# ShenhanQian/GaussianAvatars

Measured on NVIDIA H100. Metric: rasterizer fwd+bwd frames/sec @100k splats 1080p, higher is better.
Workload: dtype f32

## Files before the change

gaussianavatars_b200/build.py:

```python
from __future__ import annotations

import os
import subprocess
import sys
from concurrent.futures import ThreadPoolExecutor

HERE = os.path.dirname(os.path.abspath(__file__))
CSRC = os.path.join(HERE, "csrc")
LIB = os.path.join(HERE, "libgaussianavatars_b200.so")
OBJ_DIR = os.path.join(HERE, "csrc", "_obj")

ARCH = ["-gencode", "arch=compute_90a,code=sm_90a"]
COMMON = ["-O3", "-std=c++17", "-lineinfo", "-Xcompiler", "-fPIC", "--expt-relaxed-constexpr"]
SOURCES = {
    "api.cu": [],
    "preprocess.cu": ["--fmad=false"],
    "preprocess_bwd.cu": [],
    "binning.cu": [],
    "tile_sort.cu": [],
    "densify.cu": [],
    "regularize.cu": [],
    "nvls.cu": [],
    "blend.cu": [],
    "face_frame.cu": [],
    "flame.cu": [],
    "loss.cu": [],
    "metrics.cu": [],
    "mesh.cu": ["--fmad=false"],
    "optim.cu": [],
}


def _nvcc():
    for cand in (os.environ.get("NVCC"), "/usr/local/cuda/bin/nvcc", "nvcc"):
        if cand and (os.path.isabs(cand) and os.path.exists(cand) or not os.path.isabs(cand)):
            return cand
    return "nvcc"


def _newest_header():
    inc = [os.path.join(CSRC, f) for f in os.listdir(CSRC) if f.endswith((".cuh", ".h", ".inc"))]
    inc.append(os.path.join(HERE, "..", "include", "gab200_rasterizer.h"))
    return max(os.path.getmtime(p) for p in inc)


def build_native(force: bool = False, verbose: bool = False) -> str:
    os.makedirs(OBJ_DIR, exist_ok=True)
    hdr_time = _newest_header()
    jobs = []
    for src, extra in SOURCES.items():
        s = os.path.join(CSRC, src)
        o = os.path.join(OBJ_DIR, src.replace(".cu", ".o"))
        stale = force or not os.path.exists(o) or os.path.getmtime(o) < max(os.path.getmtime(s), hdr_time)
        if stale:
            cmd = [_nvcc(), *ARCH, *COMMON, *extra, "-ccbin", "/usr/bin/g++", "-c", s, "-o", o]
            if verbose:
                cmd.insert(1, "-Xptxas")
                cmd.insert(2, "-v")
            jobs.append(cmd)

    def run(cmd):
        r = subprocess.run(cmd, capture_output=True, text=True)
        if r.returncode != 0:
            raise RuntimeError("nvcc failed: %s\n%s\n%s" % (" ".join(cmd), r.stdout, r.stderr))
        return r.stderr

    if jobs:
        with ThreadPoolExecutor(max_workers=len(jobs)) as ex:
            for out in ex.map(run, jobs):
                if verbose and out:
                    print(out)
    objs = [os.path.join(OBJ_DIR, s.replace(".cu", ".o")) for s in SOURCES]
# ... 10 lines not shown
```

gaussianavatars_b200/csrc/api.cu:

```cuda
#include <atomic>
#include <chrono>
#include <cstdio>
#include <cstdlib>
#include <cstring>
#include <mutex>
#include <vector>

#include "common.cuh"
#include "kernels.cuh"

namespace gab {
static std::atomic<int64_t> g_launches{0};
void count_launch() { g_launches.fetch_add(1, std::memory_order_relaxed); }

struct SortTempCache {
  int64_t n = -1;
  int bits = -1;
  size_t bytes = 0;
};
static thread_local SortTempCache t_sort_cache[2];
static size_t cached_sort_temp_bytes(int64_t N, int bits) {
  SortTempCache& c = t_sort_cache[bits == 32 ? 0 : 1];
  if (c.bits != bits || N > c.n) {
    const int64_t n_up = N + N / 2 + 1024;
    c.bytes = sort_temp_bytes(n_up, bits);
    c.n = n_up;
    c.bits = bits;
  }
  return c.bytes;
}

struct GeomView {
  SplatRec* rec;
  SplatAux* aux;
  uint32_t* tiles_touched;
  uint32_t* offsets;
  uint8_t* clamped;
  uint32_t* depth_keys[2];
  uint32_t* ids[2];
  void* sortA_temp;
  size_t sortA_temp_bytes;
  float* g2d;
  float* face_scratch;
  void* scan_temp;
  size_t scan_temp_bytes;
  DepthBuckets buckets;
  size_t bucket_clear_bytes;
  size_t bytes;
};
static uint32_t depth_bucket_count(int P) {
  uint32_t nb = 256;
  while (nb < 8192 && (int64_t)nb * 64 < P) nb <<= 1;
  return nb;
}
static GeomView carve_geom(void* base, int P, bool need_backward, size_t sort_temp, int face_rows = -1) {
  GeomView g;
  Carver c(base);
  g.rec = c.take<SplatRec>((size_t)P);
  g.aux = c.take<SplatAux>((size_t)P);
  g.tiles_touched = c.take<uint32_t>((size_t)P);
  g.offsets = c.take<uint32_t>((size_t)P);
  g.clamped = c.take<uint8_t>((size_t)P);
  g.depth_keys[0] = c.take<uint32_t>((size_t)P);
  g.depth_keys[1] = c.take<uint32_t>((size_t)P);
  g.ids[0] = c.take<uint32_t>((size_t)P);
  g.ids[1] = c.take<uint32_t>((size_t)P);
  g.g2d = need_backward ? c.take<float>((size_t)P * GAB_G2D_STRIDE) : nullptr;
  g.face_scratch =
      need_backward ? c.take<float>((size_t)(face_rows < 0 ? P : face_rows) * GAB_FACE_GRAD_STRIDE) : nullptr;
  g.scan_temp_bytes = scan_temp_bytes(P);
  g.scan_temp = c.take<char>(g.scan_temp_bytes);
  {
    DepthBuckets& d = g.buckets;
    d.nb = depth_bucket_count(P);
    uint32_t* head = c.take<uint32_t>((size_t)2 * d.nb + GAB_DEPTH_META_WORDS);
    d.counts = head;
    d.tiles = head ? head + d.nb : nullptr;
    d.meta = head ? head + 2 * d.nb : nullptr;
    g.bucket_clear_bytes = sizeof(uint32_t) * ((size_t)2 * d.nb + GAB_DEPTH_META_WORDS);
    d.start = c.take<uint32_t>((size_t)d.nb);
    d.tile_base = c.take<uint32_t>((size_t)d.nb);
    d.rank = c.take<uint32_t>((size_t)P);
    d.lo = d.hi = 0;
    d.scale = 0.f;
    d.enabled = 0;
  }
  g.sortA_temp_bytes = sort_temp;
  g.sortA_temp = c.take<char>(sort_temp);
  g.bytes = c.bytes();
  return g;
}
struct BinView {
  uint32_t* keys[2];
  uint32_t* vals[2];
  uint8_t* strip_mask;
  void* sort_temp;
  size_t sort_temp_bytes;
  size_t bytes;
};
static BinView carve_binning(void* base, int64_t N, bool need_backward, size_t sort_temp) {
  BinView b;
  Carver c(base);
  const size_t n = (size_t)(N > 0 ? N : 1) + 320;
  b.keys[0] = c.take<uint32_t>(n);
  b.keys[1] = c.take<uint32_t>(n);
  b.vals[0] = c.take<uint32_t>(n);
  b.vals[1] = c.take<uint32_t>(n);
  b.strip_mask = need_backward ? c.take<uint8_t>(n) : nullptr;
  b.sort_temp_bytes = sort_temp;
  b.sort_temp = c.take<char>(sort_temp);
  b.bytes = c.bytes();
  return b;
}
struct ImageView {
  uint2* ranges;
  uint32_t* order;
  uint32_t* order_info;
  uint32_t* tile_count;
  uint32_t* tile_cursor;
  float* final_T;
  uint32_t* n_contrib;
  size_t bytes;
};
static ImageView carve_image(void* base, int W, int H, bool need_backward, int views = 1) {
  ImageView v;
  Carver c(base);
  const int gx = (W + GAB_TILE - 1) / GAB_TILE, gy = (H + GAB_TILE - 1) / GAB_TILE;
  const size_t tiles = (size_t)gx * gy * views;
  v.ranges = c.take<uint2>(tiles + 1);
  v.order = c.take<uint32_t>(tiles);
  v.order_info = c.take<uint32_t>(4);
  v.tile_count = c.take<uint32_t>(tiles);
  v.tile_cursor = c.take<uint32_t>(tiles);
  v.final_T = need_backward ? c.take<float>((size_t)W * H * views) : nullptr;
  v.n_contrib = need_backward ? c.take<uint32_t>((size_t)W * H * views) : nullptr;
  v.bytes = c.bytes();
  return v;
}

struct StageTimer {
  std::atomic<int> enabled{0};
  std::mutex mu;
  struct Pending { int stage; cudaEvent_t a, b; };
  std::vector<Pending> pending;
  std::vector<cudaEvent_t> pool;
  double total_ms[GAB200_NUM_STAGES] = {0};
  int64_t launches[GAB200_NUM_STAGES] = {0};
  cudaEvent_t get() {
    if (!pool.empty()) { cudaEvent_t e = pool.back(); pool.pop_back(); return e; }
    cudaEvent_t e; cudaEventCreate(&e); return e;
  }
};
static StageTimer g_timer;
static thread_local bool t_capturing = false;
struct StageScope {
  int stage; cudaStream_t stream; cudaEvent_t a{}, b{}; bool on;
  StageScope(int st, cudaStream_t s) : stage(st), stream(s), on(g_timer.enabled.load() != 0 && !t_capturing) {
    if (on) {
      std::lock_guard<std::mutex> l(g_timer.mu);
      a = g_timer.get(); b = g_timer.get();
      cudaEventRecord(a, stream);
    }
  }
// ... 192 lines not shown
    GAB_CUDA(cudaMemsetAsync(d.counts, 0, g.bucket_clear_bytes, stream));
    if (f.counting) GAB_CUDA(cudaMemsetAsync(f.iv.tile_count, 0, sizeof(uint32_t) * (size_t)tiles, stream));
    StageScope sc(GAB200_STAGE_PREPROCESS, stream);
    if (f.cameras != nullptr)
      launch_preprocess_views(*a, f.views, f.cameras, g.rec, g.aux, g.tiles_touched, g.depth_keys[0], g.ids[0],
                              g.buckets, f.counting ? f.iv.tile_count : nullptr, f.nb ? g.clamped : nullptr, stream);
    else
      launch_preprocess(*a, g.rec, g.aux, g.tiles_touched, f.nb ? g.clamped : nullptr, g.depth_keys[0], g.ids[0],
                        g.buckets, f.counting ? f.iv.tile_count : nullptr, f.tanfov, stream);
  }
  GAB_STAGE_CHECK(f.dbg, stream);
  if (f.counting && run_preprocess) {
    StageScope sc(GAB200_STAGE_TILE_RANGES, stream);
    f.scan_clamp = capacity > 0 ? capacity : 0xffffffffu;
    launch_tile_scan_order(tiles, f.iv.tile_count, f.scan_clamp, f.iv.ranges, f.iv.tile_cursor, f.iv.order,
                           f.iv.order_info, g.buckets.meta, tune_get(GAB200_TUNE_HEAVY_FWD),
                           tune_get(GAB200_TUNE_HEAVY_BWD), stream);
  }
  {
    StageScope sc(GAB200_STAGE_SCAN, stream);
    if (bucket) {
      launch_depth_bucket_sort(f.P, g.buckets, g.depth_keys[0], g.tiles_touched, g.depth_keys[1], g.ids[1], g.offsets,
                               capacity, a->frame_seq, a->sync_mode == GAB200_SYNC_NONE ? a->overflow_flag : nullptr,
                               stream);
      f.selA = 1;
      f.order_count = g.buckets.meta + GAB200_CTR_NUM_LISTED;
    } else {
      GAB_CUDA(run_sort(g.sortA_temp, g.sortA_temp_bytes, g.depth_keys[0], g.depth_keys[1], g.ids[0], g.ids[1], f.P, 32,
                        &f.selA, stream));
      if (!f.counting)
        GAB_CUDA(run_scan(g.scan_temp, g.scan_temp_bytes, g.ids[f.selA], g.tiles_touched, g.offsets, f.P, stream));
      f.order_count = nullptr;
    }
    if (!bucket)
      launch_publish_counters(g.buckets.meta, f.counting ? nullptr : g.offsets, f.P, capacity, a->frame_seq,
                              a->sync_mode == GAB200_SYNC_NONE ? a->overflow_flag : nullptr, stream);
  }
  GAB_STAGE_CHECK(f.dbg, stream);
  GAB_CUDA(cudaMemcpyAsync(f.ctr_host, g.buckets.meta, sizeof(uint32_t) * GAB200_NUM_COUNTERS, cudaMemcpyDeviceToHost,
                           stream));
  if (f.ctr_event) GAB_CUDA(cudaEventRecord(f.ctr_event, stream));
  return GAB200_OK;
}

void emit(const Frame& f, const uint32_t* offsets, uint32_t cap, uint32_t* cursor, const BinView& bv) {
  if (f.cameras != nullptr)
    launch_emit_keys_views(f.P, f.gx, f.gy, f.g.rec, f.g.aux, f.g.ids[f.selA], offsets, f.order_count, f.g.buckets.meta,
                           cap, cursor, bv.keys[0], bv.vals[0], f.a->exact_binning, f.a->P, f.stream);
  else
    launch_emit_keys(f.P, f.gx, f.gy, f.g.rec, f.g.aux, f.g.ids[f.selA], offsets, f.order_count, f.g.buckets.meta, cap,
                     cursor, bv.keys[0], bv.vals[0], f.a->exact_binning, f.stream);
}

int enqueue_binning_blend(Frame& f, void* bin, int64_t cap, int64_t n_known, size_t sort_temp, bool redo) {
  const gab200_forward_args* a = f.a;
  gab200_frame_state* st = f.st;
  cudaStream_t stream = f.stream;
  const int tiles = f.tiles;
  BinView bv = carve_binning(bin, cap, f.nb, sort_temp);
  st->binning_capacity = cap;
  st->binning_buffer = bin;
  st->binning_bytes = bv.bytes;
  const int64_t n_sort = n_known >= 0 ? n_known : cap;
  const bool counting = f.counting && f.P > 0;
  st->tile_sort_path = counting ? 1 : 0;
  if (bv.strip_mask != nullptr && n_sort > 0) GAB_CUDA(cudaMemsetAsync(bv.strip_mask, 0, (size_t)n_sort, stream));
  int selector = 0;
  if (counting) {
    if (redo) {
      StageScope sc(GAB200_STAGE_TILE_RANGES, stream);
      f.scan_clamp = (uint32_t)(cap < 0xffffffffll ? cap : 0xffffffffll);
      launch_tile_scan_order(tiles, f.iv.tile_count, f.scan_clamp, f.iv.ranges, f.iv.tile_cursor, f.iv.order,
                             f.iv.order_info, f.g.buckets.meta, tune_get(GAB200_TUNE_HEAVY_FWD),
                             tune_get(GAB200_TUNE_HEAVY_BWD), stream);
    }
    if (n_sort > 0) {
      {
        StageScope sc(GAB200_STAGE_EMIT_KEYS, stream);
        emit(f, nullptr, (uint32_t)cap, f.iv.tile_cursor, bv);
      }
      GAB_STAGE_CHECK(f.dbg, stream);
      {
        StageScope sc(GAB200_STAGE_SORT, stream);
        launch_tile_sort(tiles, f.iv.ranges, f.iv.order, f.iv.order_info, bv.keys[0], bv.vals[0], f.g.ids[f.selA],
                         f.order_count, f.P, stream);
      }
      GAB_STAGE_CHECK(f.dbg, stream);
    }
  } else {
    GAB_CUDA(cudaMemsetAsync(f.iv.ranges, 0, sizeof(uint2) * ((size_t)tiles + 1), stream));
    if (n_sort > 0) {
      if (n_known < 0) GAB_CUDA(cudaMemsetAsync(bv.keys[0], 0xff, sizeof(uint32_t) * (size_t)cap, stream));
      {
        StageScope sc(GAB200_STAGE_EMIT_KEYS, stream);
        emit(f, f.g.offsets, (uint32_t)cap, nullptr, bv);
      }
      GAB_STAGE_CHECK(f.dbg, stream);
      {
        StageScope sc(GAB200_STAGE_SORT, stream);
        GAB_CUDA(run_sort(bv.sort_temp, bv.sort_temp_bytes, bv.keys[0], bv.keys[1], bv.vals[0], bv.vals[1], n_sort,
                          st->sort_bits, &selector, stream));
      }
      GAB_STAGE_CHECK(f.dbg, stream);
      {
        StageScope sc(GAB200_STAGE_TILE_RANGES, stream);
        launch_tile_ranges(n_sort, (uint32_t)tiles, bv.keys[selector], f.iv.ranges, stream);
      }
      GAB_STAGE_CHECK(f.dbg, stream);
    }
    StageScope sc(GAB200_STAGE_TILE_RANGES, stream);
    launch_tile_scan_order(tiles, nullptr, 0xffffffffu, f.iv.ranges, nullptr, f.iv.order, f.iv.order_info, nullptr,
                           tune_get(GAB200_TUNE_HEAVY_FWD), tune_get(GAB200_TUNE_HEAVY_BWD), stream);
  }
  st->sorted_selector = selector;
  {
    StageScope sc(GAB200_STAGE_BLEND_FWD, stream);
    if (f.cameras != nullptr && f.nb)
      launch_blend_forward_views_train(f.views, f.W, f.H, f.iv.ranges, f.iv.order, f.iv.order_info, bv.vals[selector],
                                       f.g.rec, a->bg, a->out_color, f.iv.final_T, f.iv.n_contrib, bv.strip_mask,
                                       stream);
    else if (f.cameras != nullptr)
      launch_blend_forward_views(f.views, f.W, f.H, f.iv.ranges, f.iv.order, f.iv.order_info, bv.vals[selector], f.g.rec,
                                 a->bg, a->out_color, f.out_rgb8, stream);
    else
      launch_blend_forward(f.W, f.H, f.iv.ranges, f.iv.order, f.iv.order_info, bv.vals[selector], f.g.rec, a->bg,
                           a->out_color, f.iv.final_T, f.iv.n_contrib, bv.strip_mask, f.out_rgb8, stream);
  }
  GAB_STAGE_CHECK(f.dbg, stream);
  return GAB200_OK;
}

int wait_counters(Frame& f) {
  for (;;) {
    const cudaError_t q = cudaEventQuery(f.ctr_event);
    if (q == cudaSuccess) return GAB200_OK;
    if (q != cudaErrorNotReady) return GAB200_ERR_CUDA;
  }
}
}

static int64_t run_forward(const gab200_forward_args* a, const float* tanfov, uint8_t* out_rgb8,
                           gab200_frame_state* st, void* stream_, int views = 1, const float* cameras = nullptr) {
  cudaStream_t stream = (cudaStream_t)stream_;
  if (!validate(a, out_rgb8 != nullptr && a != nullptr && a->need_backward == 0) || st == nullptr)
    return GAB200_ERR_INVALID_ARGUMENT;
  if (check_arch() < 0) return GAB200_ERR_ARCH;
  memset(st, 0, sizeof(*st));
  Frame f;
  f.a = a; f.tanfov = tanfov; f.out_rgb8 = out_rgb8; f.st = st; f.stream = stream;
  f.P = a->P * views; f.W = a->image_width; f.H = a->image_height;
  f.gx = (f.W + GAB_TILE - 1) / GAB_TILE; f.gy = (f.H + GAB_TILE - 1) / GAB_TILE;
  f.tiles = f.gx * f.gy * views;
  f.views = views; f.cameras = cameras;
  f.nb = a->need_backward != 0;
  f.dbg = a->debug != 0;
  f.counting = tune_get(GAB200_TUNE_TILE_SORT) == 1;
  const int P = f.P;
  const int mode = a->sync_mode;
  const bool speculative = mode != GAB200_SYNC_EXACT;
  if (speculative && P > 0 && a->binning_hint <= 0) return GAB200_ERR_INVALID_ARGUMENT;
  if (mode == GAB200_SYNC_NONE && a->counters_host == nullptr) return GAB200_ERR_INVALID_ARGUMENT;
  cudaStreamCaptureStatus cap_status = cudaStreamCaptureStatusNone;
  GAB_CUDA(cudaStreamIsCapturing(stream, &cap_status));
  if (cap_status != cudaStreamCaptureStatusNone && mode != GAB200_SYNC_NONE) return GAB200_ERR_INVALID_ARGUMENT;
  struct CaptureGuard {
    bool prev;
    explicit CaptureGuard(bool c) : prev(t_capturing) { t_capturing = c; }
    ~CaptureGuard() { t_capturing = prev; }
  } capture_guard(cap_status != cudaStreamCaptureStatusNone);

  const size_t tempA = cached_sort_temp_bytes(P > 0 ? P : 1, 32);
  GeomView gsz = carve_geom(nullptr, P, f.nb, tempA, a->P);
  void* geom = a->alloc_geom(a->alloc_user, gsz.bytes);
  if (geom == nullptr) return GAB200_ERR_ALLOC;
  f.g = carve_geom(geom, P, f.nb, tempA, a->P);
  ImageView isz = carve_image(nullptr, f.W, f.H, f.nb, views);
  void* img = a->alloc_image(a->alloc_user, isz.bytes);
  if (img == nullptr) return GAB200_ERR_ALLOC;
  f.iv = carve_image(img, f.W, f.H, f.nb, views);
  st->geom_buffer = geom; st->geom_bytes = f.g.bytes;
  st->image_buffer = img; st->image_bytes = f.iv.bytes;
  st->sort_bits = (int)tile_bits((uint32_t)f.tiles);
  st->depth_bits = 32;
  st->device_counters = f.g.buckets.meta;
  st->attempts = 1;
  st->depth_key_min = 1; st->depth_key_max = 0;
  st->reserved0 = (cameras != nullptr && f.nb) ? views : 0;

  const double t0 = now_us();
  if (P == 0) {
    BinView bsz = carve_binning(nullptr, 0, f.nb, 0);
    void* bin = a->alloc_binning(a->alloc_user, bsz.bytes);
    if (bin == nullptr) return GAB200_ERR_ALLOC;
    GAB_CUDA(cudaMemsetAsync(f.g.buckets.counts, 0, f.g.bucket_clear_bytes, stream));
    const int rc = enqueue_binning_blend(f, bin, 0, 0, 0, false);
    if (rc < 0) return rc;
    st->num_rendered = st->num_candidates = 0;
    return 0;
  }

  f.ctr_host = a->counters_host;
  f.ctr_event = nullptr;
  if (mode != GAB200_SYNC_NONE) {
    if (!t_slot.ok()) return GAB200_ERR_CUDA;
    f.ctr_event = t_slot.ev;
    if (f.ctr_host == nullptr) f.ctr_host = t_slot.host;
  }
  bool bucket = a->depth_hint_hi > a->depth_hint_lo && tune_get(GAB200_TUNE_DEPTH_SORT) == 0;
  int64_t cap = speculative ? (int64_t)a->binning_hint : 0;
  int rc = enqueue_geometry(f, bucket, true, (uint32_t)cap);
  if (rc < 0) return rc;

  void* bin = nullptr;
  int64_t bin_cap = 0;
  size_t tempB = 0;
  double t_alloc = now_us();
  host_add(0, t_alloc - t0);
  if (a->binning_hint > 0) {
    bin_cap = a->binning_hint;
    tempB = f.counting ? 0 : cached_sort_temp_bytes(bin_cap, st->sort_bits);
    const BinView hv = carve_binning(nullptr, bin_cap, f.nb, tempB);
    bin = a->alloc_binning(a->alloc_user, hv.bytes);
    if (bin == nullptr) return GAB200_ERR_ALLOC;
  }
  double t1 = now_us();
  host_add(2, t1 - t_alloc);
  if (speculative) {
    rc = enqueue_binning_blend(f, bin, cap, -1, tempB, false);
    if (rc < 0) return rc;
    const double t2 = now_us();
    host_add(3, t2 - t1);
    t1 = t2;
  }
  st->depth_sort_path = bucket ? 1 : 0;
  if (mode == GAB200_SYNC_NONE) {
    st->num_rendered = st->num_candidates = -1;
    g_host_ns[5].fetch_add(1, std::memory_order_relaxed);
    return 0;
  }

  rc = wait_counters(f);
  if (rc < 0) return rc;
  bool redo = !speculative;
  if (bucket && f.ctr_host[GAB200_CTR_BUCKET_OVERFLOW] != 0) {
    bucket = false;
    st->depth_sort_path = 2;
    st->attempts++;
    rc = enqueue_geometry(f, false, false, (uint32_t)cap);
    if (rc < 0) return rc;
    rc = wait_counters(f);
    if (rc < 0) return rc;
    redo = true;
  }
  if (f.ctr_host[GAB200_CTR_NUM_RENDERED_HI] != 0) return GAB200_ERR_OVERFLOW;
  const int64_t N = (int64_t)f.ctr_host[GAB200_CTR_NUM_RENDERED];
  st->depth_key_min = ~f.ctr_host[GAB200_CTR_NOT_MIN_DEPTH_KEY];
  st->depth_key_max = f.ctr_host[GAB200_CTR_MAX_DEPTH_KEY];
  st->num_rendered = st->num_candidates = N;
  double t2 = now_us();
  host_add(1, t2 - t1);
  if (speculative && N > cap) {
    redo = true;
    st->attempts++;
  }
  if (redo) {
    if (bin == nullptr || N > bin_cap) {
      bin_cap = N;
      tempB = f.counting ? 0 : cached_sort_temp_bytes(bin_cap > 0 ? bin_cap : 1, st->sort_bits);
      const BinView bsz = carve_binning(nullptr, bin_cap, f.nb, tempB);
      bin = a->alloc_binning(a->alloc_user, bsz.bytes);
      if (bin == nullptr) return GAB200_ERR_ALLOC;
    }
    const double t3 = now_us();
    host_add(2, t3 - t2);
    rc = enqueue_binning_blend(f, bin, bin_cap, N, tempB, speculative);
    if (rc < 0) return rc;
    host_add(3, now_us() - t3);
  }
  g_host_ns[5].fetch_add(1, std::memory_order_relaxed);
  return N;
}

int64_t gab200_forward(const gab200_forward_args* a, gab200_frame_state* st, void* stream) {
  return run_forward(a, nullptr, nullptr, st, stream);
}

int64_t gab200_forward_device_fov(const gab200_forward_args* a, const float* tanfov, gab200_frame_state* st,
                                  void* stream) {
  return run_forward(a, tanfov, nullptr, st, stream);
}

int64_t gab200_forward_display(const gab200_forward_args* a, const float* tanfov, uint8_t* out_rgb8,
                               gab200_frame_state* st, void* stream) {
  return run_forward(a, tanfov, out_rgb8, st, stream);
}

int64_t gab200_forward_views(const gab200_forward_args* a, int32_t views, const float* cameras, uint8_t* out_rgb8,
                             gab200_frame_state* st, void* stream) {
  if (a == nullptr || a->need_backward != 0 || views < 1 || views > 65535 || cameras == nullptr || st == nullptr)
    return GAB200_ERR_INVALID_ARGUMENT;
  gab200_forward_args v = *a;
  v.viewmatrix = v.projmatrix = v.campos = cameras;
  if (!validate(&v, out_rgb8 != nullptr)) return GAB200_ERR_INVALID_ARGUMENT;
  const int64_t view_tiles = (((int64_t)v.image_width + GAB_TILE - 1) / GAB_TILE) *
                             (((int64_t)v.image_height + GAB_TILE - 1) / GAB_TILE);
  if ((int64_t)views * v.P > INT32_MAX || (int64_t)views * view_tiles > INT32_MAX) return GAB200_ERR_INVALID_ARGUMENT;
  return run_forward(&v, nullptr, out_rgb8, st, stream, views, cameras);
}

static bool validate_views_train(const gab200_forward_args* a, int32_t views, const float* cameras,
                                 gab200_forward_args& v) {
  if (a == nullptr || views < 1 || views > 65535 || cameras == nullptr) return false;
  v = *a;
  v.viewmatrix = v.projmatrix = v.campos = cameras;
  v.need_backward = 1;
  if (!validate(&v)) return false;
  if (v.input_mode != GAB200_INPUT_BOUND_RAW || v.colors_precomp != nullptr) return false;
  const int64_t view_tiles = (((int64_t)v.image_width + GAB_TILE - 1) / GAB_TILE) *
                             (((int64_t)v.image_height + GAB_TILE - 1) / GAB_TILE);
  return (int64_t)views * v.P <= INT32_MAX && (int64_t)views * view_tiles <= INT32_MAX;
}
// ... 429 lines not shown
```

gaussianavatars_b200/csrc/kernels.cuh:

```cuda
#pragma once
#include "common.cuh"

namespace gab {

#define SH_C0 0.28209479177387814f
#define SH_C1 0.4886025119029199f
#define SH_C2_0 1.0925484305920792f
#define SH_C2_1 -1.0925484305920792f
#define SH_C2_2 0.31539156525252005f
#define SH_C2_3 -1.0925484305920792f
#define SH_C2_4 0.5462742152960396f
#define SH_C3_0 -0.5900435899266435f
#define SH_C3_1 2.890611442640554f
#define SH_C3_2 -0.4570457994644658f
#define SH_C3_3 0.3731763325901154f
#define SH_C3_4 -0.4570457994644658f
#define SH_C3_5 1.445305721320277f
#define SH_C3_6 -0.5900435899266435f

void count_launch();
int tune_get(int knob);

struct TileSpan {
  bool any, full;
// ... 27 lines not shown
    if (ystar >= lo && ystar <= hi) xl = -dxmax;
    else xl = fminf((-B * lo - hl) / A, (-B * hi - hh) / A);
    const float X0 = px + xl - 0.02f, X1 = px + xr + 0.02f;
    int t0 = (int)ceilf((X0 - (float)(GAB_TILE - 1)) * (1.0f / GAB_TILE));
    int t1 = (int)floorf(X1 * (1.0f / GAB_TILE)) + 1;
    cx0 = min(max(t0, rx0), rx1);
    cx1 = max(min(t1, rx1), cx0);
  }
};

#define GAB_DEPTH_BUCKET_CAP 2048
#define GAB_DEPTH_META_WORDS (GAB200_NUM_COUNTERS + 2)
#define GAB_META_TOTAL64 GAB200_NUM_COUNTERS
struct DepthBuckets {
  uint32_t* counts;
  uint32_t* tiles;
  uint32_t* meta;
  uint32_t* start;
  uint32_t* tile_base;
  uint32_t* rank;
  uint32_t nb;
  uint32_t lo, hi;
  float scale;
  int enabled;
};
__device__ __forceinline__ uint32_t depth_bucket(uint32_t key, const DepthBuckets& d) {
  if (key <= d.lo) return 0u;
  if (key >= d.hi) return d.nb - 1u;
  const uint32_t b = (uint32_t)(__uint2float_rz(key - d.lo) * d.scale);
  return b < d.nb ? b : d.nb - 1u;
}
void launch_preprocess(const gab200_forward_args& a, SplatRec* rec, SplatAux* aux, uint32_t* tiles_touched,
                       uint8_t* clamped, uint32_t* depth_keys, uint32_t* ids, const DepthBuckets& buckets,
                       uint32_t* tile_count, const float* tanfov, cudaStream_t stream);
void launch_preprocess_views(const gab200_forward_args& a, int views, const float* cameras, SplatRec* rec, SplatAux* aux,
                             uint32_t* tiles_touched, uint32_t* depth_keys, uint32_t* ids, const DepthBuckets& buckets,
                             uint32_t* tile_count, uint8_t* clamped, cudaStream_t stream);
void launch_depth_bucket_sort(int P, const DepthBuckets& buckets, const uint32_t* depth_keys,
                              const uint32_t* tiles_touched, uint32_t* scratch_keys, uint32_t* sorted_ids,
                              uint32_t* offsets, uint32_t capacity, uint32_t seq, uint32_t* sticky_overflow,
                              cudaStream_t stream);
void launch_bind_activate(const gab200_forward_args& a, float* means3D, float* opacities, float* scales, float* cov3D,
                          cudaStream_t stream);
void launch_mark_visible(int P, const float* means3D, const float* V, uint8_t* present, cudaStream_t stream);
void launch_publish_counters(uint32_t* counters, const uint32_t* offsets, int P, uint32_t capacity, uint32_t seq,
                             uint32_t* sticky_overflow, cudaStream_t stream);
void launch_emit_keys(int P, int gx, int gy, const SplatRec* rec, const SplatAux* aux, const uint32_t* order,
                      const uint32_t* offsets, const uint32_t* order_count, const uint32_t* counters, uint32_t capacity,
                      uint32_t* cursor, uint32_t* keys, uint32_t* vals, int exact_binning, cudaStream_t stream);
void launch_emit_keys_views(int P, int gx, int gy, const SplatRec* rec, const SplatAux* aux, const uint32_t* order,
                            const uint32_t* offsets, const uint32_t* order_count, const uint32_t* counters, uint32_t cap,
                            uint32_t* cursor, uint32_t* keys, uint32_t* vals, int exact_binning, int view_splats,
                            cudaStream_t stream);
void launch_tile_ranges(int64_t N, uint32_t tiles, const uint32_t* keys, uint2* ranges, cudaStream_t stream);
void launch_expand_keys(int64_t N, const uint32_t* tile_keys, const uint32_t* ids, const SplatAux* aux, uint64_t* out,
                        cudaStream_t stream);
#define GAB_TILE_SORT_SMEM 2048
void launch_tile_scan_order(int tiles, const uint32_t* tile_count, uint32_t clamp, uint2* ranges, uint32_t* cursor,
                            uint32_t* order, uint32_t* order_info, uint32_t* counters, int heavy_fwd, int heavy_bwd,
                            cudaStream_t stream);
void launch_tile_sort(int tiles, const uint2* ranges, const uint32_t* order, const uint32_t* order_info, uint32_t* keys,
                      uint32_t* vals, const uint32_t* rank_to_id, const uint32_t* listed, int P, cudaStream_t stream);
void launch_expand_keys_by_range(int tiles, const uint2* ranges, const uint32_t* ids, const SplatAux* aux, uint64_t* out,
                                 cudaStream_t stream);

size_t scan_temp_bytes(int P);
cudaError_t run_scan(void* temp, size_t temp_bytes, const uint32_t* order, const uint32_t* tiles_touched, uint32_t* out,
                     int P, cudaStream_t stream);
size_t sort_temp_bytes(int64_t N, int end_bit);
cudaError_t run_sort(void* temp, size_t temp_bytes, uint32_t* keys_a, uint32_t* keys_b, uint32_t* vals_a,
                     uint32_t* vals_b, int64_t N, int end_bit, int* selector_out, cudaStream_t stream);

void launch_blend_forward(int W, int H, const uint2* ranges, const uint32_t* order, const uint32_t* order_info,
                          const uint32_t* point_list, const SplatRec* rec,
                          const float* bg, float* out_color, float* final_T, uint32_t* n_contrib, uint8_t* strip_mask,
                          uint8_t* out_rgb8, cudaStream_t stream);
void launch_blend_forward_views(int views, int W, int H, const uint2* ranges, const uint32_t* order,
                                const uint32_t* order_info, const uint32_t* point_list, const SplatRec* rec,
                                const float* bg, float* out_color, uint8_t* out_rgb8, cudaStream_t stream);
void launch_blend_forward_views_train(int views, int W, int H, const uint2* ranges, const uint32_t* order,
                                      const uint32_t* order_info, const uint32_t* point_list, const SplatRec* rec,
                                      const float* bg, float* out_color, float* final_T, uint32_t* n_contrib,
                                      uint8_t* strip_mask, cudaStream_t stream);
void launch_blend_backward(int W, int H, const uint2* ranges, const uint32_t* order, const uint32_t* order_info,
                           const uint32_t* point_list, const SplatRec* rec,
                           const float* bg, const float* final_T, const uint32_t* n_contrib, const float* dL_dpix,
                           const uint8_t* strip_mask, float* g2d, cudaStream_t stream);
void launch_blend_backward_views(int views, int W, int H, const uint2* ranges, const uint32_t* order,
                                 const uint32_t* order_info, const uint32_t* point_list, const SplatRec* rec,
                                 const float* bg, const float* final_T, const uint32_t* n_contrib, const float* dL_dpix,
                                 const uint8_t* strip_mask, float* g2d, cudaStream_t stream);

void launch_preprocess_backward(const gab200_backward_args& b, const SplatRec* rec, const SplatAux* aux,
                                const uint8_t* clamped, const float* g2d, float* face_scratch, const float* tanfov,
                                cudaStream_t stream);
void launch_preprocess_backward_views(const gab200_backward_args& b, int views, const float* cameras,
                                      const SplatAux* aux, const uint8_t* clamped, const float* g2d,
                                      float* face_scratch, cudaStream_t stream);
#define GAB_FACE_GRAD_STRIDE 13

void launch_face_frame_forward(int F, const float* verts, const int32_t* faces, float* fc, float* fR, float* fs,
                               cudaStream_t stream);
void launch_face_frame_backward(int F, const float* verts, const int32_t* faces, const float* g_fc, const float* g_fR,
                                const float* g_fs, float* g_verts, cudaStream_t stream);

void launch_l1_loss_u8(int64_t n, const float* img, const uint8_t* gt, const float* upstream, float* grad, float* loss,
                       cudaStream_t stream);

void launch_photometric_loss(int C, int H, int W, const float* img, const void* gt, int gt_is_u8, float lambda,
                             float* grad, float* loss, float* scratch, cudaStream_t stream);

size_t metrics_scratch_bytes(int H, int W);
void launch_image_metrics(int H, int W, int kind, const void* render, const uint8_t* gt, const int32_t* row, int rows,
                          const int32_t* skip, float* table, void* scratch, cudaStream_t stream);

size_t mesh_scratch_bytes(int F, int W, int H);
cudaError_t launch_mesh_render(const gab200_mesh_args& a, cudaStream_t stream);
// ... 26 lines not shown
```

gaussianavatars_b200/csrc/preprocess.cu:

```cuda
#include "common.cuh"
#include "kernels.cuh"
#include "splat_math.cuh"

namespace gab {

#define REC_SCALE_AC (-0.5f * 1.4426950408889634f)
#define REC_SCALE_B (-1.4426950408889634f)

__device__ __forceinline__ void stage_camera(const gab200_forward_args& a, Camera& cam) {
  int t = threadIdx.x;
  if (t < 16) cam.V[t] = a.viewmatrix[t];
  else if (t < 32) cam.Pm[t - 16] = a.projmatrix[t - 16];
  else if (t < 35) cam.campos[t - 32] = a.campos[t - 32];
  __syncthreads();
}
__device__ __forceinline__ void stage_camera_row(const float* __restrict__ row, Camera& cam) {
  int t = threadIdx.x;
  if (t < 16) cam.V[t] = row[t];
  else if (t < 32) cam.Pm[t - 16] = row[t];
  else if (t < 35) cam.campos[t - 32] = row[t];
  __syncthreads();
}

template <bool BOUND, bool DEVFOV>
// ... 410 lines not shown
                                                              uint32_t* __restrict__ cursor,
                                                              uint32_t* __restrict__ keys, uint32_t* __restrict__ vals,
                                                              int exact_binning, uint32_t view_splats,
                                                              uint32_t view_tiles) {
  emit_keys<true>(P, gx, gy, rec, aux, order, offsets, order_count, counters, cap, cursor, keys, vals, exact_binning,
                  view_splats, view_tiles);
}

__global__ void publish_counters_kernel(uint32_t* __restrict__ counters, const uint32_t* __restrict__ offsets, int P,
                                        uint32_t capacity, uint32_t seq, uint32_t* __restrict__ sticky_overflow) {
  if (P > 0) {
    if (offsets != nullptr) counters[GAB200_CTR_NUM_RENDERED] = offsets[P - 1];
    counters[GAB200_CTR_NUM_LISTED] = (uint32_t)P;
    counters[GAB200_CTR_BUCKET_OVERFLOW] = 0;
  }
  counters[GAB200_CTR_CAPACITY] = capacity;
  counters[GAB200_CTR_SEQ] = seq;
  const uint32_t hi = counters[GAB_META_TOTAL64 + 1];
  counters[GAB200_CTR_NUM_RENDERED_HI] = hi;
  if (sticky_overflow != nullptr &&
      (hi != 0 || counters[GAB200_CTR_BUCKET_OVERFLOW] != 0 || counters[GAB200_CTR_NUM_RENDERED] > capacity))
    *sticky_overflow = 1u;
}
void launch_publish_counters(uint32_t* counters, const uint32_t* offsets, int P, uint32_t capacity, uint32_t seq,
                             uint32_t* sticky_overflow, cudaStream_t stream) {
  publish_counters_kernel<<<1, 1, 0, stream>>>(counters, offsets, P, capacity, seq, sticky_overflow);
  count_launch();
}

void launch_emit_keys(int P, int gx, int gy, const SplatRec* rec, const SplatAux* aux, const uint32_t* order,
                      const uint32_t* offsets, const uint32_t* order_count, const uint32_t* counters, uint32_t cap,
                      uint32_t* cursor, uint32_t* keys, uint32_t* vals, int exact_binning, cudaStream_t stream) {
  const int warps = (P + 31) / 32;
  const int threads = 256, blocks = (warps * 32 + threads - 1) / threads;
  if (blocks == 0) return;
  emit_keys_kernel<<<blocks, threads, 0, stream>>>(P, gx, gy, rec, aux, order, offsets, order_count, counters, cap, cursor,
                                                   keys, vals, exact_binning);
  count_launch();
}

void launch_emit_keys_views(int P, int gx, int gy, const SplatRec* rec, const SplatAux* aux, const uint32_t* order,
                            const uint32_t* offsets, const uint32_t* order_count, const uint32_t* counters, uint32_t cap,
                            uint32_t* cursor, uint32_t* keys, uint32_t* vals, int exact_binning, int view_splats,
                            cudaStream_t stream) {
  const int warps = (P + 31) / 32;
  const int threads = 256, blocks = (warps * 32 + threads - 1) / threads;
  if (blocks == 0) return;
  emit_keys_views_kernel<<<blocks, threads, 0, stream>>>(P, gx, gy, rec, aux, order, offsets, order_count, counters, cap,
                                                         cursor, keys, vals, exact_binning, (uint32_t)view_splats,
                                                         (uint32_t)(gx * gy));
  count_launch();
}

__global__ void __launch_bounds__(256) tile_ranges_kernel(int64_t N, uint32_t tiles, const uint32_t* __restrict__ keys,
                                                          uint2* __restrict__ ranges) {
  const int64_t idx = (int64_t)blockIdx.x * blockDim.x + threadIdx.x;
  if (idx >= N) return;
  const uint32_t cur = min(keys[idx], tiles);
  if (idx == 0)
    ranges[cur].x = 0;
  else {
    const uint32_t prev = min(keys[idx - 1], tiles);
    if (cur != prev) {
      ranges[prev].y = (uint32_t)idx;
      ranges[cur].x = (uint32_t)idx;
    }
  }
  if (idx == N - 1) ranges[cur].y = (uint32_t)N;
}

__global__ void expand_keys_kernel(int64_t N, const uint32_t* __restrict__ tile_keys, const uint32_t* __restrict__ ids,
                                   const SplatAux* __restrict__ aux, uint64_t* __restrict__ out) {
  const int64_t i = (int64_t)blockIdx.x * blockDim.x + threadIdx.x;
  if (i >= N) return;
  out[i] = ((uint64_t)tile_keys[i] << 32) | (uint64_t)__float_as_uint(aux[ids[i]].depth);
}
void launch_expand_keys(int64_t N, const uint32_t* tile_keys, const uint32_t* ids, const SplatAux* aux, uint64_t* out,
                        cudaStream_t stream) {
  if (N == 0) return;
  expand_keys_kernel<<<(unsigned)((N + 255) / 256), 256, 0, stream>>>(N, tile_keys, ids, aux, out);
  count_launch();
}

void launch_tile_ranges(int64_t N, uint32_t tiles, const uint32_t* keys, uint2* ranges, cudaStream_t stream) {
  if (N == 0) return;
  const int threads = 256;
  const int64_t blocks = (N + threads - 1) / threads;
  tile_ranges_kernel<<<(unsigned)blocks, threads, 0, stream>>>(N, tiles, keys, ranges);
  count_launch();
}

}
```

include/gab200_rasterizer.h:

```cpp
#ifndef GAB200_RASTERIZER_H
#define GAB200_RASTERIZER_H

#include <stddef.h>
#include <stdint.h>

#ifdef __cplusplus
extern "C" {
#endif

#define GAB200_ABI_VERSION 3

typedef enum gab200_status {
  GAB200_OK = 0,
  GAB200_ERR_INVALID_ARGUMENT = -1,
  GAB200_ERR_CUDA = -2,
  GAB200_ERR_ALLOC = -3,
  GAB200_ERR_ARCH = -4,
  GAB200_ERR_OVERFLOW = -5
} gab200_status;

typedef enum gab200_input_mode {
  GAB200_INPUT_ACTIVATED = 0,
  GAB200_INPUT_BOUND_RAW = 1
} gab200_input_mode;
// ... 305 lines not shown
int32_t gab200_densify_apply(const gab200_densify_args* args, const gab200_densify_out* out, void* stream);

#define GAB200_FLAME_J 5
#define GAB200_FLAME_POSE_BASIS 36
#define GAB200_FLAME_MAX_EXPR 100
#define GAB200_FLAME_FRAME_FLOATS 128
typedef struct gab200_flame_assets {
  uint32_t abi_version;
  int32_t V, n_shape, n_expr, J;
  int32_t parents[GAB200_FLAME_J];
  const float* v_template;
  const float* shapedirs;
  const float* posedirs;
  const float* J_regressor;
  const float* lbs_weights;
} gab200_flame_assets;

size_t gab200_flame_scratch_bytes(int32_t V, int32_t n_expr);

int32_t gab200_flame_prepare(const gab200_flame_assets* assets, const float* shape, const float* static_offset,
                             void* scratch, void* stream);

typedef struct gab200_flame_frame_args {
  uint32_t abi_version;
  int32_t T;
  const gab200_flame_assets* assets;
  const void* scratch;
  const int32_t* timestep;
  const float* expr;
  const float* rotation;
  const float* neck_pose;
  const float* jaw_pose;
  const float* eyes_pose;
  const float* translation;
  float* frame;
} gab200_flame_frame_args;

int32_t gab200_flame_forward(const gab200_flame_frame_args* args, float* verts, float* verts_cano, void* stream);

typedef struct gab200_flame_grads {
  float* expr;
  float* rotation;
  float* neck_pose;
  float* jaw_pose;
  float* eyes_pose;
  float* translation;
} gab200_flame_grads;
int32_t gab200_flame_backward(const gab200_flame_frame_args* args, const float* dL_dverts, const float* dL_dverts_cano,
                              const gab200_flame_grads* grads, void* stream);

int32_t gab200_export_binning(const gab200_forward_args* args, const gab200_frame_state* state, uint64_t* keys,
                              uint32_t* values, uint32_t* ranges, void* stream);

enum {
  GAB200_STAGE_PREPROCESS = 0,
  GAB200_STAGE_SCAN = 1,
  GAB200_STAGE_EMIT_KEYS = 2,
  GAB200_STAGE_SORT = 3,
  GAB200_STAGE_TILE_RANGES = 4,
  GAB200_STAGE_BLEND_FWD = 5,
  GAB200_STAGE_BLEND_BWD = 6,
  GAB200_STAGE_PREPROCESS_BWD = 7,
  GAB200_NUM_STAGES = 8
};
void gab200_stage_timing_enable(int32_t enable);
void gab200_host_times(double out[6], int32_t reset);
int32_t gab200_stage_times(double total_ms[GAB200_NUM_STAGES], int64_t launches[GAB200_NUM_STAGES], int32_t reset);

enum {
  GAB200_TUNE_HEAVY_FWD = 0,
  GAB200_TUNE_HEAVY_BWD = 1,
  GAB200_TUNE_DEPTH_SORT = 2,
  GAB200_TUNE_TILE_SORT = 4,
  GAB200_TUNE_NVLS_CTAS = 5,
  GAB200_NUM_TUNABLES = 8
};
int32_t gab200_tune(int32_t knob, int32_t value);

int64_t gab200_launch_count(void);

const char* gab200_status_string(int32_t status);
uint32_t gab200_abi_version(void);

#ifdef __cplusplus
}
#endif
#endif
```

Before: 1720.

## Replace CUB tile-key sort with device-count-driven onesweep radix sort

Adds a custom onesweep-style LSD radix sort: one histogram kernel counts all digits, then each pass ranks keys with warp match-any, scatters them locally in shared memory and uses decoupled look-back for global offsets. Every kernel reads the true rendered count from the device counters, so work scales with the actual key count instead of the allocated capacity. This removes the 0xff memset of the key buffer, and the strip-mask clear is folded into the tile-ranges kernel. In exchange, the look-back spin-waits on chunks taken through an atomic counter, and the status scratch grows with capacity.

```diff
diff --git a/gaussianavatars_b200/build.py b/gaussianavatars_b200/build.py
--- a/gaussianavatars_b200/build.py
+++ b/gaussianavatars_b200/build.py
@@ -18,6 +18,7 @@
     "preprocess_bwd.cu": [],
     "binning.cu": [],
     "tile_sort.cu": [],
+    "tile_bin.cu": [],
     "densify.cu": [],
     "regularize.cu": [],
     "nvls.cu": [],
diff --git a/gaussianavatars_b200/csrc/api.cu b/gaussianavatars_b200/csrc/api.cu
--- a/gaussianavatars_b200/csrc/api.cu
+++ b/gaussianavatars_b200/csrc/api.cu
@@ -15,17 +15,15 @@
 
 struct SortTempCache {
   int64_t n = -1;
-  int bits = -1;
   size_t bytes = 0;
 };
-static thread_local SortTempCache t_sort_cache[2];
-static size_t cached_sort_temp_bytes(int64_t N, int bits) {
-  SortTempCache& c = t_sort_cache[bits == 32 ? 0 : 1];
-  if (c.bits != bits || N > c.n) {
+static thread_local SortTempCache t_sort_cache;
+static size_t cached_sort_temp_bytes(int64_t N) {
+  SortTempCache& c = t_sort_cache;
+  if (N > c.n) {
     const int64_t n_up = N + N / 2 + 1024;
-    c.bytes = sort_temp_bytes(n_up, bits);
+    c.bytes = sort_temp_bytes(n_up, 32);
     c.n = n_up;
-    c.bits = bits;
   }
   return c.bytes;
 }
@@ -94,11 +92,10 @@
   uint32_t* keys[2];
   uint32_t* vals[2];
   uint8_t* strip_mask;
-  void* sort_temp;
-  size_t sort_temp_bytes;
+  void* sort_scratch;
   size_t bytes;
 };
-static BinView carve_binning(void* base, int64_t N, bool need_backward, size_t sort_temp) {
+static BinView carve_binning(void* base, int64_t N, bool need_backward, size_t sort_scratch) {
   BinView b;
   Carver c(base);
   const size_t n = (size_t)(N > 0 ? N : 1) + 320;
@@ -107,8 +104,7 @@
   b.vals[0] = c.take<uint32_t>(n);
   b.vals[1] = c.take<uint32_t>(n);
   b.strip_mask = need_backward ? c.take<uint8_t>(n) : nullptr;
-  b.sort_temp_bytes = sort_temp;
-  b.sort_temp = c.take<char>(sort_temp);
+  b.sort_scratch = c.take<char>(sort_scratch);
   b.bytes = c.bytes();
   return b;
 }
@@ -407,21 +403,21 @@
                      cursor, bv.keys[0], bv.vals[0], f.a->exact_binning, f.stream);
 }
 
-int enqueue_binning_blend(Frame& f, void* bin, int64_t cap, int64_t n_known, size_t sort_temp, bool redo) {
+int enqueue_binning_blend(Frame& f, void* bin, int64_t cap, int64_t n_known, size_t sort_scratch, bool redo) {
   const gab200_forward_args* a = f.a;
   gab200_frame_state* st = f.st;
   cudaStream_t stream = f.stream;
   const int tiles = f.tiles;
-  BinView bv = carve_binning(bin, cap, f.nb, sort_temp);
+  BinView bv = carve_binning(bin, cap, f.nb, sort_scratch);
   st->binning_capacity = cap;
   st->binning_buffer = bin;
   st->binning_bytes = bv.bytes;
   const int64_t n_sort = n_known >= 0 ? n_known : cap;
   const bool counting = f.counting && f.P > 0;
   st->tile_sort_path = counting ? 1 : 0;
-  if (bv.strip_mask != nullptr && n_sort > 0) GAB_CUDA(cudaMemsetAsync(bv.strip_mask, 0, (size_t)n_sort, stream));
   int selector = 0;
   if (counting) {
+    if (bv.strip_mask != nullptr && n_sort > 0) GAB_CUDA(cudaMemsetAsync(bv.strip_mask, 0, (size_t)n_sort, stream));
     if (redo) {
       StageScope sc(GAB200_STAGE_TILE_RANGES, stream);
       f.scan_clamp = (uint32_t)(cap < 0xffffffffll ? cap : 0xffffffffll);
@@ -445,7 +441,6 @@
   } else {
     GAB_CUDA(cudaMemsetAsync(f.iv.ranges, 0, sizeof(uint2) * ((size_t)tiles + 1), stream));
     if (n_sort > 0) {
-      if (n_known < 0) GAB_CUDA(cudaMemsetAsync(bv.keys[0], 0xff, sizeof(uint32_t) * (size_t)cap, stream));
       {
         StageScope sc(GAB200_STAGE_EMIT_KEYS, stream);
         emit(f, f.g.offsets, (uint32_t)cap, nullptr, bv);
@@ -453,13 +448,13 @@
       GAB_STAGE_CHECK(f.dbg, stream);
       {
         StageScope sc(GAB200_STAGE_SORT, stream);
-        GAB_CUDA(run_sort(bv.sort_temp, bv.sort_temp_bytes, bv.keys[0], bv.keys[1], bv.vals[0], bv.vals[1], n_sort,
-                          st->sort_bits, &selector, stream));
+        GAB_CUDA(launch_tile_bin_sort(bv.keys, bv.vals, f.g.buckets.meta, n_sort, st->sort_bits, bv.sort_scratch,
+                                      &selector, stream));
       }
       GAB_STAGE_CHECK(f.dbg, stream);
       {
         StageScope sc(GAB200_STAGE_TILE_RANGES, stream);
-        launch_tile_ranges(n_sort, (uint32_t)tiles, bv.keys[selector], f.iv.ranges, stream);
+        launch_tile_bin_ranges(bv.keys[selector], f.g.buckets.meta, n_sort, f.iv.ranges, bv.strip_mask, stream);
       }
       GAB_STAGE_CHECK(f.dbg, stream);
     }
@@ -524,7 +519,7 @@
     ~CaptureGuard() { t_capturing = prev; }
   } capture_guard(cap_status != cudaStreamCaptureStatusNone);
 
-  const size_t tempA = cached_sort_temp_bytes(P > 0 ? P : 1, 32);
+  const size_t tempA = cached_sort_temp_bytes(P > 0 ? P : 1);
   GeomView gsz = carve_geom(nullptr, P, f.nb, tempA, a->P);
   void* geom = a->alloc_geom(a->alloc_user, gsz.bytes);
   if (geom == nullptr) return GAB200_ERR_ALLOC;
@@ -573,7 +568,7 @@
   host_add(0, t_alloc - t0);
   if (a->binning_hint > 0) {
     bin_cap = a->binning_hint;
-    tempB = f.counting ? 0 : cached_sort_temp_bytes(bin_cap, st->sort_bits);
+    tempB = f.counting ? 0 : tile_bin_scratch_bytes(bin_cap, st->sort_bits);
     const BinView hv = carve_binning(nullptr, bin_cap, f.nb, tempB);
     bin = a->alloc_binning(a->alloc_user, hv.bytes);
     if (bin == nullptr) return GAB200_ERR_ALLOC;
@@ -621,7 +616,7 @@
   if (redo) {
     if (bin == nullptr || N > bin_cap) {
       bin_cap = N;
-      tempB = f.counting ? 0 : cached_sort_temp_bytes(bin_cap > 0 ? bin_cap : 1, st->sort_bits);
+      tempB = f.counting ? 0 : tile_bin_scratch_bytes(bin_cap, st->sort_bits);
       const BinView bsz = carve_binning(nullptr, bin_cap, f.nb, tempB);
       bin = a->alloc_binning(a->alloc_user, bsz.bytes);
       if (bin == nullptr) return GAB200_ERR_ALLOC;
diff --git a/gaussianavatars_b200/csrc/kernels.cuh b/gaussianavatars_b200/csrc/kernels.cuh
--- a/gaussianavatars_b200/csrc/kernels.cuh
+++ b/gaussianavatars_b200/csrc/kernels.cuh
@@ -103,7 +103,6 @@
                             const uint32_t* offsets, const uint32_t* order_count, const uint32_t* counters, uint32_t cap,
                             uint32_t* cursor, uint32_t* keys, uint32_t* vals, int exact_binning, int view_splats,
                             cudaStream_t stream);
-void launch_tile_ranges(int64_t N, uint32_t tiles, const uint32_t* keys, uint2* ranges, cudaStream_t stream);
 void launch_expand_keys(int64_t N, const uint32_t* tile_keys, const uint32_t* ids, const SplatAux* aux, uint64_t* out,
                         cudaStream_t stream);
 #define GAB_TILE_SORT_SMEM 2048
@@ -114,6 +113,12 @@
                       uint32_t* vals, const uint32_t* rank_to_id, const uint32_t* listed, int P, cudaStream_t stream);
 void launch_expand_keys_by_range(int tiles, const uint2* ranges, const uint32_t* ids, const SplatAux* aux, uint64_t* out,
                                  cudaStream_t stream);
+
+size_t tile_bin_scratch_bytes(int64_t cap, int bits);
+cudaError_t launch_tile_bin_sort(uint32_t* keys[2], uint32_t* vals[2], const uint32_t* counters, int64_t cap, int bits,
+                                 void* scratch, int* selector_out, cudaStream_t stream);
+void launch_tile_bin_ranges(const uint32_t* keys, const uint32_t* counters, int64_t cap, uint2* ranges,
+                            uint8_t* strip_mask, cudaStream_t stream);
 
 size_t scan_temp_bytes(int P);
 cudaError_t run_scan(void* temp, size_t temp_bytes, const uint32_t* order, const uint32_t* tiles_touched, uint32_t* out,
diff --git a/gaussianavatars_b200/csrc/preprocess.cu b/gaussianavatars_b200/csrc/preprocess.cu
--- a/gaussianavatars_b200/csrc/preprocess.cu
+++ b/gaussianavatars_b200/csrc/preprocess.cu
@@ -486,23 +486,6 @@
   count_launch();
 }
 
-__global__ void __launch_bounds__(256) tile_ranges_kernel(int64_t N, uint32_t tiles, const uint32_t* __restrict__ keys,
-                                                          uint2* __restrict__ ranges) {
-  const int64_t idx = (int64_t)blockIdx.x * blockDim.x + threadIdx.x;
-  if (idx >= N) return;
-  const uint32_t cur = min(keys[idx], tiles);
-  if (idx == 0)
-    ranges[cur].x = 0;
-  else {
-    const uint32_t prev = min(keys[idx - 1], tiles);
-    if (cur != prev) {
-      ranges[prev].y = (uint32_t)idx;
-      ranges[cur].x = (uint32_t)idx;
-    }
-  }
-  if (idx == N - 1) ranges[cur].y = (uint32_t)N;
-}
-
 __global__ void expand_keys_kernel(int64_t N, const uint32_t* __restrict__ tile_keys, const uint32_t* __restrict__ ids,
                                    const SplatAux* __restrict__ aux, uint64_t* __restrict__ out) {
   const int64_t i = (int64_t)blockIdx.x * blockDim.x + threadIdx.x;
@@ -516,12 +499,4 @@
   count_launch();
 }
 
-void launch_tile_ranges(int64_t N, uint32_t tiles, const uint32_t* keys, uint2* ranges, cudaStream_t stream) {
-  if (N == 0) return;
-  const int threads = 256;
-  const int64_t blocks = (N + threads - 1) / threads;
-  tile_ranges_kernel<<<(unsigned)blocks, threads, 0, stream>>>(N, tiles, keys, ranges);
-  count_launch();
-}
-
-}
+}
diff --git a/gaussianavatars_b200/csrc/tile_bin.cu b/gaussianavatars_b200/csrc/tile_bin.cu
--- /dev/null
+++ b/gaussianavatars_b200/csrc/tile_bin.cu
@@ -0,0 +1,255 @@
+#include <algorithm>
+
+#include <cuda/atomic>
+
+#include "common.cuh"
+#include "kernels.cuh"
+
+namespace gab {
+
+#define TB_THREADS 256
+#define TB_WARPS (TB_THREADS / 32)
+#define TB_ITEMS 15
+#define TB_TILE (TB_THREADS * TB_ITEMS)
+#define TB_DIGIT_BITS 8
+#define TB_RADIX (1 << TB_DIGIT_BITS)
+#define TB_MAX_PASSES 4
+#define TB_HEAD_WORDS (TB_MAX_PASSES * TB_RADIX + TB_MAX_PASSES)
+
+static_assert(TB_RADIX == TB_THREADS, "one thread per digit");
+
+#define TB_AGGREGATE (1ull << 32)
+#define TB_INCLUSIVE (2ull << 32)
+
+__device__ __forceinline__ uint32_t tb_count(const uint32_t* counters, uint32_t cap) {
+  if (counters[GAB200_CTR_BUCKET_OVERFLOW] != 0 || counters[GAB200_CTR_NUM_RENDERED_HI] != 0) return 0;
+  return min(counters[GAB200_CTR_NUM_RENDERED], cap);
+}
+
+int tile_bin_passes(int bits) { return (bits + TB_DIGIT_BITS - 1) / TB_DIGIT_BITS; }
+
+int64_t tile_bin_chunks(int64_t cap) { return (cap + TB_TILE - 1) / TB_TILE; }
+
+size_t tile_bin_scratch_bytes(int64_t cap, int bits) {
+  Carver c(nullptr);
+  c.take<uint32_t>(TB_HEAD_WORDS);
+  c.take<unsigned long long>((size_t)tile_bin_passes(bits) * (size_t)tile_bin_chunks(cap) * TB_RADIX);
+  return c.bytes();
+}
+
+__global__ void __launch_bounds__(TB_THREADS) tile_bin_hist_kernel(const uint32_t* __restrict__ keys,
+                                                                   const uint32_t* __restrict__ counters, uint32_t cap,
+                                                                   int passes, uint32_t* __restrict__ hist,
+                                                                   unsigned long long* __restrict__ status,
+                                                                   uint32_t chunks) {
+  __shared__ uint32_t s_hist[TB_MAX_PASSES][TB_RADIX];
+  const uint32_t n = tb_count(counters, cap);
+  const size_t base = (size_t)blockIdx.x * TB_TILE;
+  if (base >= n) return;
+  const int t = threadIdx.x;
+  for (int p = 0; p < passes; p++) {
+    s_hist[p][t] = 0;
+    status[((size_t)p * chunks + blockIdx.x) * TB_RADIX + t] = 0ull;
+  }
+  __syncthreads();
+  const uint32_t valid = (uint32_t)min((size_t)TB_TILE, (size_t)n - base);
+  for (uint32_t j = t; j < valid; j += TB_THREADS) {
+    const uint32_t k = keys[base + j];
+    for (int p = 0; p < passes; p++) atomicAdd(&s_hist[p][(k >> (p * TB_DIGIT_BITS)) & (TB_RADIX - 1)], 1u);
+  }
+  __syncthreads();
+  for (int p = 0; p < passes; p++)
+    if (s_hist[p][t] != 0) atomicAdd(&hist[p * TB_RADIX + t], s_hist[p][t]);
+}
+
+__device__ __forceinline__ void tb_block_scan2(uint32_t& a, uint32_t& b, uint32_t (*s)[TB_WARPS]) {
+  const int lane = threadIdx.x & 31, w = threadIdx.x >> 5;
+  uint32_t ia = a, ib = b;
+#pragma unroll
+  for (int d = 1; d < 32; d <<= 1) {
+    const uint32_t na = __shfl_up_sync(0xffffffffu, ia, d), nb = __shfl_up_sync(0xffffffffu, ib, d);
+    if (lane >= d) { ia += na; ib += nb; }
+  }
+  if (lane == 31) { s[0][w] = ia; s[1][w] = ib; }
+  __syncthreads();
+  uint32_t oa = 0, ob = 0;
+  for (int k = 0; k < w; k++) { oa += s[0][k]; ob += s[1][k]; }
+  a = oa + ia - a;
+  b = ob + ib - b;
+}
+
+__global__ void __launch_bounds__(TB_THREADS) tile_bin_pass_kernel(
+    const uint32_t* __restrict__ keys_in, const uint32_t* __restrict__ vals_in, uint32_t* __restrict__ keys_out,
+    uint32_t* __restrict__ vals_out, const uint32_t* __restrict__ counters, uint32_t cap, int pass,
+    const uint32_t* __restrict__ hist, uint32_t* __restrict__ next_chunk, unsigned long long* __restrict__ status,
+    uint32_t chunks) {
+  __shared__ uint32_t s_warp[TB_WARPS][TB_RADIX];
+  __shared__ uint32_t s_keys[TB_TILE];
+  __shared__ uint32_t s_vals[TB_TILE];
+  __shared__ uint32_t s_local[TB_RADIX];
+  __shared__ uint32_t s_global[TB_RADIX];
+  __shared__ uint32_t s_scan[2][TB_WARPS];
+  __shared__ uint32_t s_chunk;
+  constexpr unsigned FULL = 0xffffffffu;
+  const int t = threadIdx.x, lane = t & 31, w = t >> 5;
+  if (t == 0) s_chunk = atomicAdd(next_chunk + pass, 1u);
+  for (int i = t; i < TB_WARPS * TB_RADIX; i += TB_THREADS) (&s_warp[0][0])[i] = 0;
+  __syncthreads();
+  const uint32_t chunk = s_chunk;
+  const uint32_t n = tb_count(counters, cap);
+  const size_t base = (size_t)chunk * TB_TILE;
+  if (base >= n) return;
+  const uint32_t valid = (uint32_t)min((size_t)TB_TILE, (size_t)n - base);
+  const int shift = pass * TB_DIGIT_BITS;
+
+  uint32_t key[TB_ITEMS], val[TB_ITEMS], rank[TB_ITEMS];
+  const uint32_t wbase = (uint32_t)w * (32 * TB_ITEMS);
+#pragma unroll
+  for (int i = 0; i < TB_ITEMS; i++) {
+    const uint32_t j = wbase + i * 32 + lane;
+    key[i] = j < valid ? keys_in[base + j] : 0u;
+    val[i] = j < valid ? vals_in[base + j] : 0u;
+  }
+  const uint32_t lt = (1u << lane) - 1u;
+#pragma unroll
+  for (int i = 0; i < TB_ITEMS; i++) {
+    const bool ok = wbase + i * 32 + lane < valid;
+    const uint32_t d = ok ? (key[i] >> shift) & (TB_RADIX - 1) : TB_RADIX;
+    const uint32_t peers = __match_any_sync(FULL, d);
+    const uint32_t before = __popc(peers & lt);
+    const uint32_t run = ok ? s_warp[w][d] : 0u;
+    __syncwarp();
+    if (ok && before == 0) s_warp[w][d] = run + __popc(peers);
+    __syncwarp();
+    rank[i] = run + before;
+  }
+  __syncthreads();
+
+  uint32_t count = 0;
+#pragma unroll
+  for (int k = 0; k < TB_WARPS; k++) {
+    const uint32_t c = s_warp[k][t];
+    s_warp[k][t] = count;
+    count += c;
+  }
+  cuda::atomic_ref<unsigned long long, cuda::thread_scope_device> mine(
+      status[((size_t)pass * chunks + chunk) * TB_RADIX + t]);
+  if (chunk == 0)
+    mine.store(TB_INCLUSIVE | count, cuda::memory_order_relaxed);
+  else
+    mine.store(TB_AGGREGATE | count, cuda::memory_order_relaxed);
+  uint32_t local = count, start = hist[pass * TB_RADIX + t];
+  tb_block_scan2(local, start, s_scan);
+  s_local[t] = local;
+  __syncthreads();
+
+#pragma unroll
+  for (int i = 0; i < TB_ITEMS; i++) {
+    if (wbase + i * 32 + lane < valid) {
+      const uint32_t d = (key[i] >> shift) & (TB_RADIX - 1);
+      const uint32_t p = s_local[d] + s_warp[w][d] + rank[i];
+      s_keys[p] = key[i];
+      s_vals[p] = val[i];
+    }
+  }
+
+  uint32_t before = 0;
+  if (chunk != 0) {
+    for (uint32_t k = chunk - 1;; k--) {
+      cuda::atomic_ref<unsigned long long, cuda::thread_scope_device> prev(
+          status[((size_t)pass * chunks + k) * TB_RADIX + t]);
+      unsigned long long s;
+      do { s = prev.load(cuda::memory_order_relaxed); } while ((s >> 32) == 0);
+      before += (uint32_t)s;
+      if ((s >> 32) == (TB_INCLUSIVE >> 32)) break;
+    }
+    mine.store(TB_INCLUSIVE | (before + count), cuda::memory_order_relaxed);
+  }
+  s_global[t] = start + before - local;
+  __syncthreads();
+
+  for (uint32_t p = t; p < valid; p += TB_THREADS) {
+    const uint32_t k = s_keys[p];
+    const uint32_t o = s_global[(k >> shift) & (TB_RADIX - 1)] + p;
+    keys_out[o] = k;
+    vals_out[o] = s_vals[p];
+  }
+}
+
+__global__ void __launch_bounds__(256) tile_bin_ranges_kernel(const uint32_t* __restrict__ keys,
+                                                              const uint32_t* __restrict__ counters, uint32_t cap,
+                                                              uint2* __restrict__ ranges,
+                                                              uint8_t* __restrict__ strip_mask) {
+  const uint32_t n = tb_count(counters, cap);
+  for (size_t idx = (size_t)blockIdx.x * blockDim.x + threadIdx.x; idx < n; idx += (size_t)gridDim.x * blockDim.x) {
+    const uint32_t cur = keys[idx];
+    if (idx == 0) {
+      ranges[cur].x = 0;
+    } else {
+      const uint32_t prev = keys[idx - 1];
+      if (cur != prev) {
+        ranges[prev].y = (uint32_t)idx;
+        ranges[cur].x = (uint32_t)idx;
+      }
+    }
+    if (idx == n - 1) ranges[cur].y = n;
+    if (strip_mask != nullptr) strip_mask[idx] = 0;
+  }
+}
+
+cudaError_t launch_tile_bin_sort(uint32_t* keys[2], uint32_t* vals[2], const uint32_t* counters, int64_t cap, int bits,
+                                 void* scratch, int* selector_out, cudaStream_t stream) {
+  const int passes = tile_bin_passes(bits);
+  *selector_out = passes & 1;
+  if (cap <= 0 || passes == 0) return cudaSuccess;
+  const int64_t chunks = tile_bin_chunks(cap);
+  Carver c(scratch);
+  uint32_t* head = c.take<uint32_t>(TB_HEAD_WORDS);
+  unsigned long long* status = c.take<unsigned long long>((size_t)passes * (size_t)chunks * TB_RADIX);
+  uint32_t* hist = head;
+  uint32_t* next_chunk = head + TB_MAX_PASSES * TB_RADIX;
+  cudaError_t e = cudaMemsetAsync(head, 0, sizeof(uint32_t) * TB_HEAD_WORDS, stream);
+  if (e != cudaSuccess) return e;
+  tile_bin_hist_kernel<<<(unsigned)chunks, TB_THREADS, 0, stream>>>(keys[0], counters, (uint32_t)cap, passes, hist,
+                                                                      status, (uint32_t)chunks);
+  count_launch();
+  for (int p = 0; p < passes; p++) {
+    tile_bin_pass_kernel<<<(unsigned)chunks, TB_THREADS, 0, stream>>>(keys[p & 1], vals[p & 1], keys[(p + 1) & 1],
+                                                                        vals[(p + 1) & 1], counters, (uint32_t)cap, p,
+                                                                        hist, next_chunk, status, (uint32_t)chunks);
+    count_launch();
+  }
+  return cudaPeekAtLastError();
+}
+
+void launch_tile_bin_ranges(const uint32_t* keys, const uint32_t* counters, int64_t cap, uint2* ranges,
+                            uint8_t* strip_mask, cudaStream_t stream) {
+  if (cap <= 0) return;
+  const int64_t blocks = std::min<int64_t>((cap + 255) / 256, (int64_t)GAB_NUM_SMS * 8);
+  tile_bin_ranges_kernel<<<(unsigned)blocks, 256, 0, stream>>>(keys, counters, (uint32_t)cap, ranges, strip_mask);
+  count_launch();
+}
+
+}
+
+extern "C" {
+
+size_t gab200_sort_by_tile_scratch_bytes(int64_t capacity, int32_t bits) {
+  if (capacity < 0 || bits < 0 || bits > 32) return 0;
+  return gab::tile_bin_scratch_bytes(capacity, bits);
+}
+
+int32_t gab200_sort_by_tile(uint32_t* keys0, uint32_t* keys1, uint32_t* vals0, uint32_t* vals1,
+                            const uint32_t* counters, int64_t capacity, int32_t bits, void* scratch, void* stream) {
+  if (capacity < 0 || capacity > 0xffffffffll || bits < 0 || bits > 32) return GAB200_ERR_INVALID_ARGUMENT;
+  if (capacity > 0 && (!keys0 || !keys1 || !vals0 || !vals1 || !counters || !scratch)) return GAB200_ERR_INVALID_ARGUMENT;
+  uint32_t* keys[2] = {keys0, keys1};
+  uint32_t* vals[2] = {vals0, vals1};
+  int selector = 0;
+  if (gab::launch_tile_bin_sort(keys, vals, counters, capacity, bits, scratch, &selector, (cudaStream_t)stream) !=
+      cudaSuccess)
+    return GAB200_ERR_CUDA;
+  return selector;
+}
+
+}
diff --git a/include/gab200_rasterizer.h b/include/gab200_rasterizer.h
--- a/include/gab200_rasterizer.h
+++ b/include/gab200_rasterizer.h
@@ -381,6 +381,10 @@
 int32_t gab200_export_binning(const gab200_forward_args* args, const gab200_frame_state* state, uint64_t* keys,
                               uint32_t* values, uint32_t* ranges, void* stream);
 
+size_t gab200_sort_by_tile_scratch_bytes(int64_t capacity, int32_t bits);
+int32_t gab200_sort_by_tile(uint32_t* keys0, uint32_t* keys1, uint32_t* vals0, uint32_t* vals1, const uint32_t* counters,
+                            int64_t capacity, int32_t bits, void* scratch, void* stream);
+
 enum {
   GAB200_STAGE_PREPROCESS = 0,
   GAB200_STAGE_SCAN = 1,
```

After: 1747, median of 6. 1.6% higher.
